# GmxMahdi/compute-raytracer

Measured on AMD Instinct MI355X. Metric: Mrays/s at 3840x2160, 1024 spheres, 8 bounces, higher is better.
Workload: dtype f32; 1 GPU; C3: 3840x2160, 1024 spheres (seed 358), 8 bounces, constant sky, reference default camera/light; mode=fast, variant=0, rays_per_frame=46143642, frames_in_flight=4, parallelism=row-tiles x1

## Files before the change

compute_raytracer_amd/abi.py:

```python
import ctypes
import os

_HERE = os.path.dirname(os.path.abspath(__file__))
LIB_PATH = os.environ.get("RT355_LIB") or os.path.join(_HERE, "librt355.so")

RT_OK = 0
RT_ERR_INVALID_ARG = -1
RT_ERR_NO_DEVICE = -2
RT_ERR_HIP = -3
RT_ERR_UNSUPPORTED = -4
RT_ERR_STATE = -5
RT_ERR_CAPACITY = -6
RT_ERR_COMM = -7
RT355_COMM_ID_BYTES = 128

RT_KERNEL_RAYTRACER = 0
RT_KERNEL_HEATMAP = 1
RT_MODE_FAST = 0
RT_MODE_STRICT = 1
RT_QUERY_LIMITS = 1

SYMBOLS = [
    "rt_create", "rt_destroy", "rt_last_error", "rt_abi_version", "rt_resize", "rt_write_params",
    "rt_write_spheres", "rt_write_cubemap_face", "rt_write_triangles", "rt_write_nodes", "rt_write_blas",
    "rt_write_tri_lookup", "rt_write_blas_lookup", "rt_write_mesh_texture", "rt_select_kernel", "rt_set_mode",
    "rt_set_variant", "rt_set_partition", "rt_tiles_of_rank", "rt_padded_tiles", "rt_render", "rt_wait",
    "rt_read_pixels", "rt_get_stats", "rt_render_to", "rt_assemble_frame", "rt_device_pixels",
    "rt_build_hierarchy", "rt_filter_plan", "rt_build_flow", "rt_order_tiles", "rt_read_hierarchy",
    "rt_comm_unique_id", "rt_comm_init", "rt_comm_destroy", "rt_render_gather", "rt_frame_pixels", "rt_read_frame",
    "rt_group_create", "rt_group_destroy", "rt_group_size", "rt_group_ctx", "rt_group_render", "rt_group_wait",
    "rt_build_id", "rt_kernel_name", "rt_set_comm_timeout",
    "rt_read_pixels_async", "rt_read_pixels_wait", "rt_host_alloc", "rt_host_free",
    "rt_trace_rays", "rt_trace_rays_host", "rt_pick",
    "rt_trace_rays_ex", "rt_trace_rays_host_ex", "rt_occluded", "rt_occluded_host",
]

KERNEL_IDS = {0: "none", 1: "literal", 2: "brute_single", 3: "brute_pipeline", 4: "hierarchy_8", 5: "hierarchy_12",
              6: "hierarchy_16", 7: "hierarchy_global", 8: "triangles", 9: "heatmap", 10: "triangles_roles"}


class RtStats(ctypes.Structure):
    _fields_ = [
        ("width", ctypes.c_uint32), ("height", ctypes.c_uint32), ("local_tiles", ctypes.c_uint32),
        ("spheres", ctypes.c_uint32), ("rays", ctypes.c_uint64), ("kernel_ms", ctypes.c_float),
        ("prep_ms", ctypes.c_float), ("frames", ctypes.c_uint32), ("mode", ctypes.c_int),
        ("batch_frames", ctypes.c_uint32), ("batch_kernel_ms", ctypes.c_float),
        ("gather_ms", ctypes.c_float), ("batch_gather_ms", ctypes.c_float),
        ("kernel_id", ctypes.c_uint32), ("grid_share", ctypes.c_uint32), ("instance_uploads", ctypes.c_uint32),
        ("tri_form", ctypes.c_uint32), ("pair_rebuilds", ctypes.c_uint32),
    ]


class RtHit(ctypes.Structure):
    _fields_ = [
        ("t", ctypes.c_float), ("u", ctypes.c_float), ("v", ctypes.c_float),
        ("prim", ctypes.c_int32), ("instance", ctypes.c_int32), ("normal", ctypes.c_float * 3),
    ]


HIT_DTYPE = [("t", "<f4"), ("u", "<f4"), ("v", "<f4"), ("prim", "<i4"), ("instance", "<i4"), ("normal", "<f4", (3,))]


class RtError(RuntimeError):
    def __init__(self, code, message):
        super().__init__("rt355 error %d: %s" % (code, message))
        self.code = code


_lib = None


def _one_hip_runtime():
    import sys
    if "torch" in sys.modules:
        return
    try:
        import importlib.util
        spec = importlib.util.find_spec("torch")
        if spec is None or not spec.submodule_search_locations:
            return
        cand = os.path.join(list(spec.submodule_search_locations)[0], "lib", "libamdhip64.so")
        if os.path.exists(cand):
            ctypes.CDLL(cand, mode=ctypes.RTLD_GLOBAL)
    except Exception:
        pass


def load():
    global _lib
    if _lib is not None:
        return _lib
    if not os.path.exists(LIB_PATH):
        raise RtError(RT_ERR_NO_DEVICE, "librt355.so is not built (%s); run `make lib`. There is no CPU path." % LIB_PATH)
    os.environ.setdefault("GPU_MAX_HW_QUEUES", "8")
    _one_hip_runtime()
    L = ctypes.CDLL(LIB_PATH)
    vp, u32, sz = ctypes.c_void_p, ctypes.c_uint32, ctypes.c_size_t
    fp = ctypes.POINTER(ctypes.c_float)
    sig = {
        "rt_create": (ctypes.c_int, [ctypes.c_int, ctypes.POINTER(vp)]),
        "rt_destroy": (ctypes.c_int, [vp]),
        "rt_last_error": (ctypes.c_char_p, [vp]),
        "rt_abi_version": (ctypes.c_int, []),
        "rt_resize": (ctypes.c_int, [vp, u32, u32]),
        "rt_write_params": (ctypes.c_int, [vp, fp]),
        "rt_write_spheres": (ctypes.c_int, [vp, fp, u32]),
        "rt_write_cubemap_face": (ctypes.c_int, [vp, ctypes.c_int, u32, u32, vp]),
        "rt_write_triangles": (ctypes.c_int, [vp, fp, u32]),
        "rt_write_nodes": (ctypes.c_int, [vp, sz, fp, u32]),
        "rt_write_blas": (ctypes.c_int, [vp, fp, u32]),
        "rt_write_tri_lookup": (ctypes.c_int, [vp, fp, u32]),
        "rt_write_blas_lookup": (ctypes.c_int, [vp, fp, u32]),
        "rt_write_mesh_texture": (ctypes.c_int, [vp, u32, u32, vp]),
        "rt_select_kernel": (ctypes.c_int, [vp, ctypes.c_int]),
        "rt_set_mode": (ctypes.c_int, [vp, ctypes.c_int]),
        "rt_set_variant": (ctypes.c_int, [vp, ctypes.c_int]),
        "rt_set_partition": (ctypes.c_int, [vp, u32, u32]),
        "rt_tiles_of_rank": (u32, [u32, u32, u32]),
        "rt_padded_tiles": (u32, [u32, u32]),
        "rt_render": (ctypes.c_int, [vp]),
        "rt_wait": (ctypes.c_int, [vp]),
        "rt_read_pixels": (ctypes.c_int, [vp, vp, sz]),
        "rt_get_stats": (ctypes.c_int, [vp, ctypes.POINTER(RtStats)]),
        "rt_render_to": (ctypes.c_int, [vp, vp, sz, vp]),
        "rt_assemble_frame": (ctypes.c_int, [vp, vp, vp, u32, vp]),
        "rt_device_pixels": (ctypes.c_int, [vp, ctypes.POINTER(vp), ctypes.POINTER(sz)]),
        "rt_build_hierarchy": (ctypes.c_int, [fp, u32, fp, ctypes.POINTER(u32), u32, ctypes.POINTER(u32)]),
        "rt_filter_plan": (ctypes.c_int, [fp, u32, fp, ctypes.POINTER(ctypes.c_int), ctypes.POINTER(ctypes.c_int)]),
        "rt_order_tiles": (ctypes.c_int, [vp, ctypes.POINTER(u32), u32, u32, ctypes.POINTER(u32), sz]),
        "rt_read_hierarchy": (ctypes.c_int, [vp, fp, ctypes.POINTER(u32), u32, ctypes.POINTER(u32)]),
        "rt_comm_unique_id": (ctypes.c_int, [vp]),
        "rt_comm_init": (ctypes.c_int, [vp, vp, u32, u32]),
        "rt_comm_destroy": (ctypes.c_int, [vp]),
        "rt_render_gather": (ctypes.c_int, [vp, ctypes.c_int]),
        "rt_frame_pixels": (ctypes.c_int, [vp, ctypes.POINTER(vp), ctypes.POINTER(sz)]),
        "rt_read_frame": (ctypes.c_int, [vp, vp, sz]),
        "rt_group_create": (ctypes.c_int, [ctypes.c_int, ctypes.POINTER(vp)]),
        "rt_group_destroy": (ctypes.c_int, [vp]),
        "rt_group_size": (ctypes.c_int, [vp]),
        "rt_group_ctx": (vp, [vp, ctypes.c_int]),
        "rt_group_render": (ctypes.c_int, [vp, ctypes.c_int]),
        "rt_group_wait": (ctypes.c_int, [vp]),
        "rt_build_id": (ctypes.c_char_p, []),
        "rt_kernel_name": (ctypes.c_char_p, [ctypes.c_int]),
        "rt_set_comm_timeout": (ctypes.c_int, [vp, u32]),
        "rt_read_pixels_async": (ctypes.c_int, [vp, u32, vp, sz]),
        "rt_read_pixels_wait": (ctypes.c_int, [vp]),
        "rt_host_alloc": (ctypes.c_int, [sz, ctypes.POINTER(vp)]),
        "rt_host_free": (ctypes.c_int, [vp]),
        "rt_trace_rays": (ctypes.c_int, [vp, vp, u32, vp, vp]),
        "rt_trace_rays_host": (ctypes.c_int, [vp, vp, u32, vp]),
        "rt_pick": (ctypes.c_int, [vp, vp, u32, vp]),
        "rt_trace_rays_ex": (ctypes.c_int, [vp, vp, u32, u32, vp, vp]),
        "rt_trace_rays_host_ex": (ctypes.c_int, [vp, vp, u32, u32, vp]),
        "rt_occluded": (ctypes.c_int, [vp, vp, u32, u32, vp, vp]),
        "rt_occluded_host": (ctypes.c_int, [vp, vp, u32, u32, vp]),
    }
    for name, (res, args) in sig.items():
        fn = getattr(L, name)
        fn.restype = res
        fn.argtypes = args
    _lib = L
    return L


def check(rc, ctx=None):
    if rc != RT_OK:
        msg = load().rt_last_error(ctx)
        raise RtError(rc, msg.decode("utf-8", "replace") if msg else "")
    return rc
```

compute_raytracer_amd/csrc/rt_api.hip:

```cpp
#include "rt_ctx.h"

#include <algorithm>
#include <cmath>
#include <condition_variable>
#include <mutex>
#include <thread>
#include <cstdio>
#include <cstdlib>
#include <cstring>
#include <new>
#include <string>
#include <vector>

#include "rt_bvh_build.h"
#include "rt_tlas_fit.h"

thread_local std::string g_rt_err;
thread_local int g_rt_kernel_id = 0;
thread_local int g_rt_tri_form = 0;

#ifndef RT355_BUILD_ID
#define RT355_BUILD_ID "unknown"
#endif

// ... 988 lines not shown
            RT_HIP(hipEventRecord(c->ev_k1[c->in_flight - 1u], st));
        }
#endif
    if (rc == RT_OK) { c->d_out = dst; c->buf_slot[k] = (int)c->in_flight - 1; ++c->frames_rendered; }
    return rc;
}

int rt_render_to(rt_ctx* c, void* device_dst, size_t cap, void* hip_stream) {
    if (!c || !device_dst) return fail(RT_ERR_INVALID_ARG, "rt_render_to: NULL argument");
    const size_t need = (size_t)local_tiles(c) * 8u * c->W * 4u;
    if (cap < need) return fail(RT_ERR_CAPACITY, "rt_render_to: destination smaller than local_tiles*8*W*4");
    hipStream_t s = hip_stream ? static_cast<hipStream_t>(hip_stream) : c->stream;
    return rt_enqueue(c, static_cast<uint8_t*>(device_dst), s);
}

void rt_abandon_in_flight(rt_ctx* c) {
    for (int k = 0; k < kStreams; ++k)
        if (c->streams[k]) (void)hipStreamSynchronize(c->streams[k]);
    if (c->in_flight) {
        (void)hipMemsetAsync(c->d_rays, 0, kCtrlBytes * c->in_flight, c->stream);
        (void)hipStreamSynchronize(c->stream);
    }
    (void)hipGetLastError();
    c->in_flight = 0;
    c->stats.batch_frames = 0;
    for (int v = 0; v < kVersions; ++v) c->ver_gen[v] = 0;
}

int rt_wait(rt_ctx* c) {
    if (!c) return fail(RT_ERR_INVALID_ARG, "rt_wait: ctx is NULL");
    RT_HIP(hipSetDevice(c->device));
    if (c->comm && c->in_flight) {
        int rc = rt_comm_wait_frames(c);
        if (rc != RT_OK) return rc;
    }
    for (uint32_t i = 0; i < c->in_flight; ++i) RT_HIP(hipEventSynchronize(c->ev_done[i]));
    if (c->in_flight) {
        c->stats.frames += c->in_flight;
        c->stats.rays = c->h_rays[2u * (c->in_flight - 1u)];
        c->stats.batch_frames = c->in_flight;
        {
            uint32_t distinct = 0;
            for (int k = 0; k < kStreams; ++k) {
                bool used = false;
                for (uint32_t i = 0; i < c->in_flight; ++i) used = used || c->slot_stream[i] == c->streams[k];
                distinct += used ? 1u : 0u;
            }
            c->pipelined_hint = distinct > 1u;
        }
        c->stats.batch_kernel_ms = 0.0f;
        for (uint32_t i = 0; i < c->in_flight; ++i) {
            float ms = 0.0f;
            if (hipEventElapsedTime(&ms, c->ev_k0[i], c->ev_k1[i]) == hipSuccess) {
                c->stats.kernel_ms = ms;
                c->stats.batch_kernel_ms += ms;
            }
            if (hipEventElapsedTime(&ms, c->ev_prep0[i], c->ev_k0[i]) == hipSuccess) c->stats.prep_ms = ms;
        }
        (void)hipGetLastError();
        c->in_flight = 0;
        for (int k = 0; k < kStreams; ++k) c->buf_slot[k] = -1;
        unsigned long long fault = 0ull;
        for (uint32_t i = 0; i < c->stats.batch_frames; ++i) fault = std::max(fault, c->h_rays[2u * i + 1u]);
        if (fault != 0ull) {
            char buf[160];
            std::snprintf(buf, sizeof buf, "rt_wait: the ray-trace kernel reported fault %llu (1: dynamic LDS not at address 0); the frame is incomplete", fault);
            g_rt_err = buf;
            return RT_ERR_HIP;
        }
        return rt_comm_after_wait(c);
    }
    return RT_OK;
}

int rt_read_pixels(rt_ctx* c, uint8_t* dst, size_t cap) {
    if (!c || !dst) return fail(RT_ERR_INVALID_ARG, "rt_read_pixels: NULL argument");
    if (!c->d_out) return fail(RT_ERR_STATE, "rt_read_pixels: no colour buffer (rt_resize first)");
    int rc = rt_wait(c);
    if (rc != RT_OK) return rc;
    const uint32_t lt = local_tiles(c);
    size_t rows = 0;
    for (uint32_t j = 0; j < lt; ++j) {
        const uint32_t y0 = (c->rank + j * c->world) * 8u;
        rows += (c->H - y0 >= 8u) ? 8u : (c->H - y0);
    }
    const size_t need = rows * c->W * 4u;
    if (cap < need) return fail(RT_ERR_CAPACITY, "rt_read_pixels: destination smaller than the local rows * W * 4");
    RT_HIP(hipMemcpyAsync(dst, c->d_out, need, hipMemcpyDeviceToHost, c->stream));
    RT_HIP(hipStreamSynchronize(c->stream));
    return RT_OK;
}

int rt_read_pixels_async(rt_ctx* c, uint32_t frames_back, uint8_t* dst, size_t cap) {
    if (!c || !dst) return fail(RT_ERR_INVALID_ARG, "rt_read_pixels_async: NULL argument");
    if (frames_back >= (uint32_t)kStreams || frames_back >= c->frames_rendered)
        return fail(RT_ERR_INVALID_ARG, "rt_read_pixels_async: frames_back must name one of the last four rt_render calls");
    if (c->world != 1u || c->comm) return fail(RT_ERR_STATE, "rt_read_pixels_async: whole-frame contexts only");
    if (!c->d_outs[0]) return fail(RT_ERR_STATE, "rt_read_pixels_async: no colour buffer (rt_resize first)");
    const size_t need = (size_t)c->H * c->W * 4u;
    if (cap < need) return fail(RT_ERR_CAPACITY, "rt_read_pixels_async: destination smaller than H * W * 4");
    RT_HIP(hipSetDevice(c->device));
    const uint32_t k = (c->frames_rendered - 1u - frames_back) % (uint32_t)kStreams;
    if (c->buf_slot[k] >= 0) RT_HIP(hipStreamWaitEvent(c->copy_stream, c->ev_k1[c->buf_slot[k]], 0));
    RT_HIP(hipMemcpyAsync(dst, c->d_outs[k], need, hipMemcpyDeviceToHost, c->copy_stream));
    RT_HIP(hipEventRecord(c->ev_copy[k], c->copy_stream));
    c->copy_pending[k] = true;
    return RT_OK;
}

int rt_read_pixels_wait(rt_ctx* c) {
    if (!c) return fail(RT_ERR_INVALID_ARG, "rt_read_pixels_wait: ctx is NULL");
    RT_HIP(hipSetDevice(c->device));
    RT_HIP(hipStreamSynchronize(c->copy_stream));
    for (int k = 0; k < kStreams; ++k) c->copy_pending[k] = false;
    return RT_OK;
}

int rt_host_alloc(size_t bytes, void** out) {
    if (!out || bytes == 0) return fail(RT_ERR_INVALID_ARG, "rt_host_alloc: NULL / zero size");
    *out = nullptr;
    RT_HIP(hipHostMalloc(out, bytes, hipHostMallocDefault));
    return RT_OK;
}

int rt_host_free(void* p) {
    if (p) RT_HIP(hipHostFree(p));
    return RT_OK;
}

int rt_get_stats(rt_ctx* c, rt_stats* out) {
    if (!c || !out) return fail(RT_ERR_INVALID_ARG, "rt_get_stats: NULL argument");
    c->stats.width = c->W;
    c->stats.height = c->H;
    c->stats.local_tiles = local_tiles(c);
    c->stats.spheres = c->n;
    c->stats.mode = c->mode;
    *out = c->stats;
    return RT_OK;
}

int rt_assemble_frame(rt_ctx* c, const void* gathered, void* frame, uint32_t world, void* hip_stream) {
    if (!c || !gathered || !frame) return fail(RT_ERR_INVALID_ARG, "rt_assemble_frame: NULL argument");
    if (world == 0) return fail(RT_ERR_INVALID_ARG, "rt_assemble_frame: world must be >= 1");
    if (!c->W || !c->H) return fail(RT_ERR_STATE, "rt_assemble_frame: rt_resize has not been called");
    RT_HIP(hipSetDevice(c->device));
    hipStream_t s = hip_stream ? static_cast<hipStream_t>(hip_stream) : c->stream;
    RT_HIP(rt_launch_assemble(static_cast<const uint8_t*>(gathered), static_cast<uint8_t*>(frame), c->W, c->H, world,
                              rt_padded_tiles(c->H, world), s));
    return RT_OK;
}

int rt_build_hierarchy(const float* records, uint32_t n, float* rec4, uint32_t* link, uint32_t cap_nodes,
                       uint32_t* n_nodes) {
    if ((n && !records) || !n_nodes) return fail(RT_ERR_INVALID_ARG, "rt_build_hierarchy: NULL argument");
    std::vector<float> r;
    std::vector<uint32_t> l;
    const uint32_t nodes = rt_bvh_build(records, n, r, l, rt_bvh_arity());
    *n_nodes = nodes;
    if (l.empty()) return RT_OK;
    if (cap_nodes < nodes + 1u || !rec4 || !link) return fail(RT_ERR_CAPACITY, "rt_build_hierarchy: need n_nodes + 1 entries");
    std::memcpy(rec4, r.data(), r.size() * sizeof(float));
    std::memcpy(link, l.data(), l.size() * sizeof(uint32_t));
    return RT_OK;
}

int rt_build_flow(const float* nodes, uint32_t n_nodes, const uint32_t* roots, uint32_t n_roots, float* pairs, uint32_t cap_pairs,
                  uint32_t* n_pairs, uint32_t* root_meta) {
    if (!nodes || (n_roots && !roots) || !n_pairs) return fail(RT_ERR_INVALID_ARG, "rt_build_flow: NULL argument");
    RtFlow f;
    rt_flow_build(nodes, n_nodes, roots, n_roots, f);
    *n_pairs = f.n_pairs;
    if (!f.ok) return fail(RT_ERR_UNSUPPORTED, "rt_build_flow: node buffer beyond 65,536 entries or a count beyond 16 bits");
    if (f.n_pairs && (cap_pairs < f.n_pairs || !pairs)) return fail(RT_ERR_CAPACITY, "rt_build_flow: need room for n_pairs records");
    if (f.n_pairs) std::memcpy(pairs, f.pairs.data(), (size_t)f.n_pairs * 64u);
    if (root_meta)
        for (uint32_t r = 0; r < n_roots; ++r)
            root_meta[r] = rt_flow_meta(nodes, n_nodes, roots[r] < n_nodes - 1u ? roots[r] : n_nodes - 1u, f.pair_of);
    return RT_OK;
}

int rt_order_tiles(rt_ctx* c, const uint32_t* cost, uint32_t n, uint32_t wave_slots, uint32_t* order, size_t cap) {
    if (!c || (n && !cost) || !order) return fail(RT_ERR_INVALID_ARG, "rt_order_tiles: NULL argument");
    if (cap < (size_t)n + 2u) return fail(RT_ERR_CAPACITY, "rt_order_tiles: order needs n + 2 entries");
    if (n > (1u << 26)) return fail(RT_ERR_INVALID_ARG, "rt_order_tiles: more than 2^26 tiles");
    order[0] = order[1] = 0u;
    if (n == 0u) return RT_OK;
    RT_HIP(hipSetDevice(c->device));
    const size_t cost_bytes = ((size_t)n * 4u + 7u) & ~(size_t)7u, scan_bytes = (size_t)rt_order_scan_words() * 4u;
    void *d_cost = nullptr, *d_order = nullptr;
    hipError_t e = hipMalloc(&d_cost, cost_bytes + scan_bytes);
    if (e == hipSuccess) e = hipMalloc(&d_order, ((size_t)n + 2u) * 4u);
    if (e == hipSuccess) e = hipMemsetAsync(d_cost, 0, cost_bytes + scan_bytes, c->stream);
    if (e == hipSuccess) e = hipMemcpyAsync(d_cost, cost, (size_t)n * 4u, hipMemcpyHostToDevice, c->stream);
    uint32_t* const scan = reinterpret_cast<uint32_t*>(static_cast<char*>(d_cost) + cost_bytes);
    for (int pass = 0; pass < 2 && e == hipSuccess; ++pass) {
        if (pass) e = hipMemcpyAsync(d_cost, cost, (size_t)n * 4u, hipMemcpyHostToDevice, c->stream);
        if (e == hipSuccess) e = rt_launch_order_hist(static_cast<uint32_t*>(d_cost), scan, static_cast<uint32_t*>(d_order), n, wave_slots, nullptr, nullptr, 0u, nullptr, c->stream);
        if (e == hipSuccess) e = rt_launch_order_scatter(static_cast<uint32_t*>(d_cost), scan, static_cast<uint32_t*>(d_order), n, c->stream);
    }
    if (e == hipSuccess) e = hipMemcpyAsync(order, d_order, ((size_t)n + 2u) * 4u, hipMemcpyDeviceToHost, c->stream);
    if (e == hipSuccess) e = hipStreamSynchronize(c->stream);
    (void)hipFree(d_cost);
    (void)hipFree(d_order);
    if (e != hipSuccess) return fail_hip(e, "rt_order_tiles");
    return RT_OK;
}

int rt_read_hierarchy(rt_ctx* c, float* rec4, uint32_t* link, uint32_t cap_nodes, uint32_t* n_nodes) {
    if (!c || !n_nodes) return fail(RT_ERR_INVALID_ARG, "rt_read_hierarchy: NULL argument");
    *n_nodes = 0;
    if (c->scene_kind != 0 || c->bvh_nodes == 0u || !c->d_bvh_rec || !c->d_bvh_link)
        return fail(RT_ERR_STATE, "rt_read_hierarchy: no frame of this sphere scene has walked a hierarchy");
    const uint32_t nodes = c->bvh_nodes;
    *n_nodes = nodes;
    if (cap_nodes < nodes + 1u || !rec4 || !link) return fail(RT_ERR_CAPACITY, "rt_read_hierarchy: need n_nodes + 1 entries");
    RT_HIP(hipSetDevice(c->device));
    { int rc = drain(c); if (rc != RT_OK) return rc; }
    const size_t nn = (size_t)nodes + 1u;
    RT_HIP(hipMemcpyAsync(rec4, c->d_bvh_rec, nn * sizeof(float4), hipMemcpyDeviceToHost, c->stream));
    RT_HIP(hipMemcpyAsync(link, c->d_bvh_link, nn * sizeof(uint32_t), hipMemcpyDeviceToHost, c->stream));
    RT_HIP(hipStreamSynchronize(c->stream));
    return RT_OK;
}

int rt_filter_plan(const float* records, uint32_t n, const float params[24], int* filter_ok, int* signed_filter) {
    if ((n && !records) || !params || !filter_ok || !signed_filter) return fail(RT_ERR_INVALID_ARG, "rt_filter_plan: NULL argument");
    bool ok = false;
    uint32_t sgn = 0;
    rt_plan((double)(float)rt_scene_bound(records, n), rt_scene_min_radius(records, n), params, ok, sgn);
    *filter_ok = ok ? 1 : 0;
    *signed_filter = (int)sgn;
    return RT_OK;
}


static int query_prepare(rt_ctx* c, const char* who, hipStream_t s, bool& tri, RtTriScene& ts, int& inst) {
    char msg[160];
    tri = c->scene_kind == 1;
    inst = 0;
    if (tri) {
        const bool have_blas = c->inst.blas_on ? !c->inst.blas.empty() : c->d_blas[0].used != 0;
        const bool have_lookup = c->inst.lookup_on ? !c->inst.lookup.empty() : c->d_blas_lookup[0].used != 0;
        if (!c->d_tri.used || !c->nodes_used || !have_blas || !c->d_tri_lookup.used || !have_lookup) {
            std::snprintf(msg, sizeof msg, "%s: a triangle scene needs rt_write_triangles, _nodes, _blas, _tri_lookup and _blas_lookup", who);
            return fail(RT_ERR_STATE, msg);
        }
    } else if (!c->have_spheres) {
        std::snprintf(msg, sizeof msg, "%s: no scene has been written", who);
        return fail(RT_ERR_STATE, msg);
    }
    RT_HIP(hipSetDevice(c->device));
    if (!c->ev_query) RT_HIP(hipEventCreateWithFlags(&c->ev_query, hipEventDisableTiming));
    if (tri) { int rc = ensure_corners(c, s); if (rc != RT_OK) return rc; }
    uint32_t v = 0;
    uint32_t root_meta[kInstMax] = {0};
    bool have_pairs = false;
    if (tri) {
        const uint32_t n_inst = (uint32_t)(c->inst.blas.size() / 20u);
        inst = (c->inst.blas_on && c->inst.lookup_on && n_inst >= 1u && c->inst.lookup.size() <= n_inst) ? 1 : 0;
        if (inst) {
            uint32_t roots[kInstMax], n_roots = 0;
            if (tri_pair_roots(c, roots, n_roots)) have_pairs = tri_pairs_current(c, roots, n_roots, root_meta);
        } else {
            int cur = -1;
            for (int k = 0; k < kVersions && cur < 0; ++k)
                if (c->ver_gen[k] == c->inst.gen) cur = k;
            if (cur < 0) {
                { int rc = drain(c); if (rc != RT_OK) return rc; }
                cur = 0;
                { int rc = apply_version(c, 0u, 0u, s); if (rc != RT_OK) return rc; }
            } else if (c->ev_ver[cur] && c->ver_stream[cur] != s) {
                RT_HIP(hipStreamWaitEvent(s, c->ev_ver[cur], 0));
            }
            v = (uint32_t)cur;
            c->query_versions = true;
        }
    }
    if (c->scene_stream && c->scene_stream != s) RT_HIP(hipStreamWaitEvent(s, c->ev_scene, 0));
    if (c->query_pending && c->query_last != s) RT_HIP(hipStreamWaitEvent(s, c->ev_query, 0));
    if (tri) {
        std::memset(&ts, 0, sizeof ts);
        tri_scene(c, v, have_pairs, root_meta, ts);
        if (inst) tri_fill_inst(c, ts);
    }
    return RT_OK;
}

static int query_launch(rt_ctx* c, const float4* rays, void* out, uint32_t n, hipStream_t s, bool tri, const RtTriScene& ts, int inst,
                        uint32_t flags = 0u, bool any = false) {
    if (!flags && !any) {
        float4* hits = static_cast<float4*>(out);
        if (tri) RT_HIP(rt_launch_query_triangles(ts, inst, rays, hits, n, s));
        else RT_HIP(rt_launch_query_spheres(c->d_records, c->n, rays, hits, n, s));
    } else {
        if (tri) RT_HIP(rt_launch_limited_triangles(ts, inst, rays, flags, any, out, n, s));
        else RT_HIP(rt_launch_limited_spheres(c->d_records, c->n, rays, flags, any, out, n, s));
    }
    RT_HIP(hipEventRecord(c->ev_query, s));
    c->query_pending = true;
    c->query_last = s;
    return RT_OK;
}

static int grow_staging(rt_ctx::DevBuf& b, size_t need) {
    if (need <= b.cap) return RT_OK;
    (void)hipFree(b.p);
    b.p = nullptr; b.cap = 0;
    const size_t cap = std::max(need, (size_t)65536u);
    RT_HIP(hipMalloc(&b.p, cap));
    b.cap = cap;
    return RT_OK;
// ... 112 lines not shown
```

compute_raytracer_amd/csrc/rt_bvh_build.h:

```cpp
#pragma once
#include <algorithm>
#include <cmath>
#include <cstdint>
#include <vector>

#ifndef RT_FILTER_KAPPA
#define RT_FILTER_KAPPA 1.52587890625e-05f
#define RT_FILTER_EPS 7.62939453125e-06f
#define RT_FILTER_SCALE 1099511627776.0f
#define RT_FILTER_SCALE2 1208925819614629174706176.0f
#endif
#ifndef RT_BVH_SIGMA
#define RT_BVH_SIGMA 1.04
#endif

namespace {

struct Builder {
    const float* rec;
    std::vector<float>& out_rec;
    std::vector<uint32_t>& out_link;
    std::vector<uint32_t> ids;
    uint32_t arity = 4;

    double cx(uint32_t i, int a) const {
        const double v = (double)rec[8u * (size_t)i + (size_t)a];
        return v == v ? v : 0.0;
    }
    double rad(uint32_t i) const {
        const double v = std::fabs((double)rec[8u * (size_t)i + 7u]);
        return v == v ? v : 0.0;
    }

    void leaf(uint32_t sphere) {
        out_rec.insert(out_rec.end(), {0.0f, 0.0f, 0.0f, 0.0f});
        out_link.push_back(0x80000000u | sphere);
    }

    uint32_t split2(uint32_t lo, uint32_t hi) {
        const uint32_t n = hi - lo;
        auto by_axis = [&](int ax) {
            return [this, ax](uint32_t a, uint32_t b) {
                const double va = cx(a, ax), vb = cx(b, ax);
                return va < vb || (va == vb && a < b);
            };
        };
        if (n > 32768u) {
            double mn[3] = {INFINITY, INFINITY, INFINITY}, mx[3] = {-INFINITY, -INFINITY, -INFINITY};
            for (uint32_t k = lo; k < hi; ++k)
                for (int a = 0; a < 3; ++a) {
                    const double v = cx(ids[k], a);
                    mn[a] = std::min(mn[a], v); mx[a] = std::max(mx[a], v);
                }
            int ax = 0;
            if (mx[1] - mn[1] > mx[ax] - mn[ax]) ax = 1;
            if (mx[2] - mn[2] > mx[ax] - mn[ax]) ax = 2;
            const uint32_t mid = lo + n / 2u;
            std::nth_element(ids.begin() + lo, ids.begin() + mid, ids.begin() + hi, by_axis(ax));
            return mid;
        }
        double best = INFINITY;
        int best_ax = 0;
        uint32_t best_k = n / 2u;
        std::vector<uint32_t> order(n);
        std::vector<double> suffix(n);
        for (int ax = 0; ax < 3; ++ax) {
            std::copy(ids.begin() + lo, ids.begin() + hi, order.begin());
            std::sort(order.begin(), order.end(), by_axis(ax));
            double mn[3] = {INFINITY, INFINITY, INFINITY}, mx[3] = {-INFINITY, -INFINITY, -INFINITY};
            auto grow = [&](uint32_t i) {
                double d2 = 0.0;
                for (int a = 0; a < 3; ++a) {
                    mn[a] = std::min(mn[a], cx(i, a) - rad(i));
                    mx[a] = std::max(mx[a], cx(i, a) + rad(i));
                    d2 += (mx[a] - mn[a]) * (mx[a] - mn[a]);
                }
                return d2;
            };
            for (uint32_t k = n; k-- > 1u;) suffix[k] = grow(order[k]) * (double)(n - k);
            for (int a = 0; a < 3; ++a) { mn[a] = INFINITY; mx[a] = -INFINITY; }
            for (uint32_t k = 1; k < n; ++k) {
                const double cost = grow(order[k - 1u]) * (double)k + suffix[k];
                if (cost < best) { best = cost; best_ax = ax; best_k = k; }
            }
        }
        std::sort(ids.begin() + lo, ids.begin() + hi, by_axis(best_ax));
        return lo + best_k;
    }

    void bound(uint32_t lo, uint32_t hi, float out[4]) {
        double mn[3] = {INFINITY, INFINITY, INFINITY}, mx[3] = {-INFINITY, -INFINITY, -INFINITY};
        for (uint32_t k = lo; k < hi; ++k)
            for (int a = 0; a < 3; ++a) {
                mn[a] = std::min(mn[a], cx(ids[k], a) - rad(ids[k]));
                mx[a] = std::max(mx[a], cx(ids[k], a) + rad(ids[k]));
            }
        auto radius_at = [&](const double P[3], uint32_t& far) {
            double R = -1.0;
            for (uint32_t k = lo; k < hi; ++k) {
                const uint32_t i = ids[k];
                const double dx = cx(i, 0) - P[0], dy = cx(i, 1) - P[1], dz = cx(i, 2) - P[2];
                const double d = std::sqrt(dx * dx + dy * dy + dz * dz) + rad(i);
                if (d > R) { R = d; far = i; }
            }
            return R;
        };
        double P[3] = {0.5 * (mn[0] + mx[0]), 0.5 * (mn[1] + mx[1]), 0.5 * (mn[2] + mx[2])};
        uint32_t far = ids[lo];
        double Rp = radius_at(P, far);
        for (int it = 0; it < 32; ++it) {
            const double s[3] = {cx(far, 0) - P[0], cx(far, 1) - P[1], cx(far, 2) - P[2]};
            const double len = std::sqrt(s[0] * s[0] + s[1] * s[1] + s[2] * s[2]);
            if (!(len > 1e-12)) break;
            const double Q[3] = {P[0] + s[0] / len * 0.05 * Rp, P[1] + s[1] / len * 0.05 * Rp, P[2] + s[2] / len * 0.05 * Rp};
            uint32_t far_q = far;
            const double Rq = radius_at(Q, far_q);
            if (!(Rq < Rp)) break;
            P[0] = Q[0]; P[1] = Q[1]; P[2] = Q[2]; Rp = Rq; far = far_q;
        }
        if (hi - lo > 2u) {
            double Q[3] = {P[0], P[1], P[2]};
            for (int it = 1; it <= 96; ++it) {
                uint32_t fq = far;
                const double Rq = radius_at(Q, fq);
                if (Rq < Rp) { Rp = Rq; P[0] = Q[0]; P[1] = Q[1]; P[2] = Q[2]; }
                const double s[3] = {cx(fq, 0) - Q[0], cx(fq, 1) - Q[1], cx(fq, 2) - Q[2]};
                const double len = std::sqrt(s[0] * s[0] + s[1] * s[1] + s[2] * s[2]);
                if (!(len > 1e-12)) break;
                const double k = (1.0 + rad(fq) / len) / (double)(it + 1);
                Q[0] += s[0] * k; Q[1] += s[1] * k; Q[2] += s[2] * k;
            }
        }
        const float C[3] = {(float)P[0], (float)P[1], (float)P[2]};
        const double Cd[3] = {C[0], C[1], C[2]};
        uint32_t unused = 0;
        double R = radius_at(Cd, unused);
        R *= RT_BVH_SIGMA;
        const double c2 = (double)C[0] * C[0] + (double)C[1] * C[1] + (double)C[2] * C[2];
        const double k = c2 * (1.0 - (double)RT_FILTER_EPS) - R * R * (1.0 + (double)RT_FILTER_KAPPA);
        out[0] = C[0] * RT_FILTER_SCALE; out[1] = C[1] * RT_FILTER_SCALE; out[2] = C[2] * RT_FILTER_SCALE;
        out[3] = (float)(k * (double)RT_FILTER_SCALE2);
    }

    void emit(uint32_t lo, uint32_t hi) {
        if (hi - lo == 1u) { leaf(ids[lo]); return; }
        const size_t me = out_link.size();
        out_rec.insert(out_rec.end(), {0.0f, 0.0f, 0.0f, 0.0f});
        out_link.push_back(0u);
        children(lo, hi);
        float b[4];
        bound(lo, hi, b);
        std::copy(b, b + 4, out_rec.begin() + 4 * me);
        out_link[me] = 4u * (uint32_t)out_link.size();
    }

    void children(uint32_t lo, uint32_t hi) {
        if (hi - lo <= arity) {
            for (uint32_t k = lo; k < hi; ++k) leaf(ids[k]);
            return;
        }
        uint32_t cut[9] = {lo, hi, 0, 0, 0, 0, 0, 0, 0};
        int parts = 1;
        while (parts < (int)arity) {
            int big = 0;
            for (int j = 1; j < parts; ++j)
                if (cut[j + 1] - cut[j] > cut[big + 1] - cut[big]) big = j;
            if (cut[big + 1] - cut[big] < 2u) break;
            const uint32_t mid = split2(cut[big], cut[big + 1]);
            for (int j = parts; j > big; --j) cut[j + 1] = cut[j];
            cut[big + 1] = mid;
            ++parts;
        }
        for (int j = 0; j < parts; ++j) emit(cut[j], cut[j + 1]);
    }
};

}

inline uint32_t rt_bvh_build(const float* records, uint32_t n, std::vector<float>& rec4, std::vector<uint32_t>& link, uint32_t arity = 4u) {
    rec4.clear(); link.clear();
    if (n == 0) return 0;
    rec4.reserve((size_t)n * 6u); link.reserve((size_t)n * 3u / 2u + 8u);
    Builder b{records, rec4, link, {}};
    b.arity = arity < 2u ? 2u : (arity > 8u ? 8u : arity);
    double mn[3] = {INFINITY, INFINITY, INFINITY}, mx[3] = {-INFINITY, -INFINITY, -INFINITY};
    for (uint32_t i = 0; i < n; ++i)
        for (int a = 0; a < 3; ++a) { mn[a] = std::min(mn[a], b.cx(i, a)); mx[a] = std::max(mx[a], b.cx(i, a)); }
    std::vector<double> radii(n);
    for (uint32_t i = 0; i < n; ++i) radii[i] = b.rad(i);
    std::nth_element(radii.begin(), radii.begin() + n / 2u, radii.end());
    const double med = radii[n / 2u];
    const double ext = std::sqrt((mx[0] - mn[0]) * (mx[0] - mn[0]) + (mx[1] - mn[1]) * (mx[1] - mn[1]) + (mx[2] - mn[2]) * (mx[2] - mn[2]));
    uint32_t big = 0;
    for (uint32_t i = 0; i < n; ++i) {
        const bool large = n > 8u && b.rad(i) > 8.0 * med && b.rad(i) > 0.125 * ext;
        if (large && big < 64u) { b.leaf(i); ++big; } else b.ids.push_back(i);
    }
    if (!b.ids.empty()) b.children(0u, (uint32_t)b.ids.size());
    const uint32_t nodes = (uint32_t)link.size();
    rec4.insert(rec4.end(), {0.0f, 0.0f, 0.0f, INFINITY});
    link.push_back(4u * nodes);
    return nodes;
}
```

include/rt355.h:

```cpp
#ifndef RT355_H
#define RT355_H

#include <stddef.h>
#include <stdint.h>

#ifdef __cplusplus
extern "C" {
#endif

#define RT355_ABI_VERSION 4

typedef enum rt_status {
    RT_OK = 0,
    RT_ERR_INVALID_ARG = -1,
    RT_ERR_NO_DEVICE = -2,
    RT_ERR_HIP = -3,
    RT_ERR_UNSUPPORTED = -4,
    RT_ERR_STATE = -5,
    RT_ERR_CAPACITY = -6,
    RT_ERR_COMM = -7
} rt_status;

typedef enum rt_kernel_id {
    RT_KID_NONE = 0,
    RT_KID_LITERAL = 1,
    RT_KID_BRUTE_SINGLE = 2,
    RT_KID_BRUTE_PIPELINE = 3,
    RT_KID_HIERARCHY_8 = 4,
    RT_KID_HIERARCHY_12 = 5,
    RT_KID_HIERARCHY_16 = 6,
    RT_KID_HIERARCHY_GLOBAL = 7,
    RT_KID_TRIANGLES = 8,
    RT_KID_HEATMAP = 9,
    RT_KID_TRIANGLES_ROLES = 10
} rt_kernel_id;

typedef enum rt_kernel {
    RT_KERNEL_RAYTRACER = 0,
    RT_KERNEL_HEATMAP = 1
} rt_kernel;

typedef enum rt_mode { RT_MODE_FAST = 0, RT_MODE_STRICT = 1 } rt_mode;

typedef struct rt_ctx rt_ctx;

typedef struct rt_stats {
    uint32_t width, height;
    uint32_t local_tiles;
    uint32_t spheres;
    uint64_t rays;
    float kernel_ms;
    float prep_ms;
    uint32_t frames;
    int mode;
    uint32_t batch_frames;
    float batch_kernel_ms;
    float gather_ms;
    float batch_gather_ms;
    uint32_t kernel_id;
    uint32_t grid_share;
    uint32_t instance_uploads;
    uint32_t tri_form;
    uint32_t pair_rebuilds;
} rt_stats;


int rt_create(int device, rt_ctx** out);
int rt_destroy(rt_ctx* ctx);

const char* rt_last_error(rt_ctx* ctx);

int rt_abi_version(void);

const char* rt_build_id(void);
const char* rt_kernel_name(int kernel_id);


int rt_resize(rt_ctx* ctx, uint32_t width, uint32_t height);

int rt_write_params(rt_ctx* ctx, const float params[24]);

int rt_write_spheres(rt_ctx* ctx, const float* records, uint32_t n);

int rt_write_cubemap_face(rt_ctx* ctx, int face, uint32_t w, uint32_t h, const uint8_t* rgba);

int rt_write_triangles(rt_ctx* ctx, const float* data, uint32_t n_triangles);
int rt_write_nodes(rt_ctx* ctx, size_t byte_offset, const float* data, uint32_t n);
int rt_write_blas(rt_ctx* ctx, const float* data, uint32_t n_blas);
int rt_write_tri_lookup(rt_ctx* ctx, const float* data, uint32_t n);
int rt_write_blas_lookup(rt_ctx* ctx, const float* data, uint32_t n);
int rt_write_mesh_texture(rt_ctx* ctx, uint32_t w, uint32_t h, const uint8_t* rgba);

int rt_select_kernel(rt_ctx* ctx, int kernel);

int rt_set_mode(rt_ctx* ctx, int mode);

int rt_set_variant(rt_ctx* ctx, int variant);


int rt_set_partition(rt_ctx* ctx, uint32_t rank, uint32_t world);

uint32_t rt_tiles_of_rank(uint32_t height, uint32_t rank, uint32_t world);
uint32_t rt_padded_tiles(uint32_t height, uint32_t world);


#define RT355_MAX_IN_FLIGHT 64
int rt_render(rt_ctx* ctx);

int rt_wait(rt_ctx* ctx);

int rt_read_pixels(rt_ctx* ctx, uint8_t* dst, size_t cap);

int rt_read_pixels_async(rt_ctx* ctx, uint32_t frames_back, uint8_t* dst, size_t cap);
int rt_read_pixels_wait(rt_ctx* ctx);
int rt_host_alloc(size_t bytes, void** out);
int rt_host_free(void* p);

int rt_get_stats(rt_ctx* ctx, rt_stats* out);


int rt_render_to(rt_ctx* ctx, void* device_dst, size_t cap, void* hip_stream);

int rt_assemble_frame(rt_ctx* ctx, const void* gathered, void* frame, uint32_t world,
                      void* hip_stream);

int rt_device_pixels(rt_ctx* ctx, void** out_ptr, size_t* out_bytes);


typedef struct rt_hit {
    float t;
    float u, v;
    int32_t prim;
    int32_t instance;
    float normal[3];
} rt_hit;

int rt_trace_rays(rt_ctx* ctx, const float* rays, uint32_t n, rt_hit* hits, void* hip_stream);
int rt_trace_rays_host(rt_ctx* ctx, const float* rays, uint32_t n, rt_hit* hits);
int rt_pick(rt_ctx* ctx, const uint32_t* xy, uint32_t n, rt_hit* hits);


#define RT_QUERY_LIMITS 1u

int rt_trace_rays_ex(rt_ctx* ctx, const float* rays, uint32_t n, uint32_t flags, rt_hit* hits, void* hip_stream);
int rt_trace_rays_host_ex(rt_ctx* ctx, const float* rays, uint32_t n, uint32_t flags, rt_hit* hits);
int rt_occluded(rt_ctx* ctx, const float* rays, uint32_t n, uint32_t flags, uint8_t* occluded, void* hip_stream);
int rt_occluded_host(rt_ctx* ctx, const float* rays, uint32_t n, uint32_t flags, uint8_t* occluded);


#define RT355_COMM_ID_BYTES 128
int rt_comm_unique_id(uint8_t id[RT355_COMM_ID_BYTES]);
int rt_comm_init(rt_ctx* ctx, const uint8_t id[RT355_COMM_ID_BYTES], uint32_t rank, uint32_t world);
int rt_comm_destroy(rt_ctx* ctx);

int rt_set_comm_timeout(rt_ctx* ctx, uint32_t ms);

int rt_render_gather(rt_ctx* ctx, int root);

int rt_frame_pixels(rt_ctx* ctx, void** out_ptr, size_t* out_bytes);
int rt_read_frame(rt_ctx* ctx, uint8_t* dst, size_t cap);

typedef struct rt_group rt_group;
int rt_group_create(int n_devices, rt_group** out);
int rt_group_destroy(rt_group* g);
int rt_group_size(const rt_group* g);
rt_ctx* rt_group_ctx(rt_group* g, int i);
int rt_group_render(rt_group* g, int root);
int rt_group_wait(rt_group* g);


int rt_build_hierarchy(const float* records, uint32_t n, float* rec4, uint32_t* link, uint32_t cap_nodes,
                       uint32_t* n_nodes);

int rt_build_flow(const float* nodes, uint32_t n_nodes, const uint32_t* roots, uint32_t n_roots, float* pairs, uint32_t cap_pairs,
                  uint32_t* n_pairs, uint32_t* root_meta);

int rt_order_tiles(rt_ctx* ctx, const uint32_t* cost, uint32_t n, uint32_t wave_slots, uint32_t* order, size_t cap);

int rt_read_hierarchy(rt_ctx* ctx, float* rec4, uint32_t* link, uint32_t cap_nodes, uint32_t* n_nodes);

int rt_filter_plan(const float* records, uint32_t n, const float params[24], int* filter_ok, int* signed_filter);

#ifdef __cplusplus
}
#endif
#endif
```

Before: 31140 Mrays/s.

## Add reinsertion optimisation pass to sphere BVH builder

After the top-down build, the BVH builder now keeps an explicit node tree and runs a reinsertion optimiser. It detaches subtrees under the largest parents, searches for cheaper placements using a bounding-ball cost, and keeps moves that lower the cost, with journaled rollback. Emitted bounds are recomputed for dirty nodes, and the result is discarded if the final cost rises. The aim is a tighter hierarchy so traversal visits fewer nodes per ray, at the price of extra host build time and more complex builder code.

```diff
diff --git a/compute_raytracer_amd/abi.py b/compute_raytracer_amd/abi.py
--- a/compute_raytracer_amd/abi.py
+++ b/compute_raytracer_amd/abi.py
@@ -33,6 +33,7 @@
     "rt_read_pixels_async", "rt_read_pixels_wait", "rt_host_alloc", "rt_host_free",
     "rt_trace_rays", "rt_trace_rays_host", "rt_pick",
     "rt_trace_rays_ex", "rt_trace_rays_host_ex", "rt_occluded", "rt_occluded_host",
+    "rt_build_hierarchy_ex",
 ]
 
 KERNEL_IDS = {0: "none", 1: "literal", 2: "brute_single", 3: "brute_pipeline", 4: "hierarchy_8", 5: "hierarchy_12",
@@ -126,6 +127,8 @@
         "rt_assemble_frame": (ctypes.c_int, [vp, vp, vp, u32, vp]),
         "rt_device_pixels": (ctypes.c_int, [vp, ctypes.POINTER(vp), ctypes.POINTER(sz)]),
         "rt_build_hierarchy": (ctypes.c_int, [fp, u32, fp, ctypes.POINTER(u32), u32, ctypes.POINTER(u32)]),
+        "rt_build_hierarchy_ex": (ctypes.c_int, [fp, u32, fp, ctypes.POINTER(u32), u32, ctypes.POINTER(u32), u32,
+                                                 ctypes.POINTER(ctypes.c_double)]),
         "rt_filter_plan": (ctypes.c_int, [fp, u32, fp, ctypes.POINTER(ctypes.c_int), ctypes.POINTER(ctypes.c_int)]),
         "rt_order_tiles": (ctypes.c_int, [vp, ctypes.POINTER(u32), u32, u32, ctypes.POINTER(u32), sz]),
         "rt_read_hierarchy": (ctypes.c_int, [vp, fp, ctypes.POINTER(u32), u32, ctypes.POINTER(u32)]),
diff --git a/compute_raytracer_amd/csrc/rt_api.hip b/compute_raytracer_amd/csrc/rt_api.hip
--- a/compute_raytracer_amd/csrc/rt_api.hip
+++ b/compute_raytracer_amd/csrc/rt_api.hip
@@ -1164,11 +1164,18 @@
 
 int rt_build_hierarchy(const float* records, uint32_t n, float* rec4, uint32_t* link, uint32_t cap_nodes,
                        uint32_t* n_nodes) {
+    return rt_build_hierarchy_ex(records, n, rec4, link, cap_nodes, n_nodes, RT355_HIERARCHY_PASSES, nullptr);
+}
+
+int rt_build_hierarchy_ex(const float* records, uint32_t n, float* rec4, uint32_t* link, uint32_t cap_nodes,
+                          uint32_t* n_nodes, uint32_t passes, double* info) {
     if ((n && !records) || !n_nodes) return fail(RT_ERR_INVALID_ARG, "rt_build_hierarchy: NULL argument");
     std::vector<float> r;
     std::vector<uint32_t> l;
-    const uint32_t nodes = rt_bvh_build(records, n, r, l, rt_bvh_arity());
+    rt_bvh_build_info bi;
+    const uint32_t nodes = rt_bvh_build(records, n, r, l, rt_bvh_arity(), passes > 16u ? 16u : passes, &bi);
     *n_nodes = nodes;
+    if (info) { info[0] = (double)bi.nodes_topdown; info[1] = (double)bi.moves; info[2] = bi.cost_topdown; info[3] = bi.cost; }
     if (l.empty()) return RT_OK;
     if (cap_nodes < nodes + 1u || !rec4 || !link) return fail(RT_ERR_CAPACITY, "rt_build_hierarchy: need n_nodes + 1 entries");
     std::memcpy(rec4, r.data(), r.size() * sizeof(float));
diff --git a/compute_raytracer_amd/csrc/rt_bvh_build.h b/compute_raytracer_amd/csrc/rt_bvh_build.h
--- a/compute_raytracer_amd/csrc/rt_bvh_build.h
+++ b/compute_raytracer_amd/csrc/rt_bvh_build.h
@@ -2,6 +2,7 @@
 #include <algorithm>
 #include <cmath>
 #include <cstdint>
+#include <utility>
 #include <vector>
 
 #ifndef RT_FILTER_KAPPA
@@ -88,7 +89,7 @@
         return lo + best_k;
     }
 
-    void bound(uint32_t lo, uint32_t hi, float out[4]) {
+    void bound(uint32_t lo, uint32_t hi, float out[4], double* sphere = nullptr) {
         double mn[3] = {INFINITY, INFINITY, INFINITY}, mx[3] = {-INFINITY, -INFINITY, -INFINITY};
         for (uint32_t k = lo; k < hi; ++k)
             for (int a = 0; a < 3; ++a) {
@@ -135,6 +136,7 @@
         const double Cd[3] = {C[0], C[1], C[2]};
         uint32_t unused = 0;
         double R = radius_at(Cd, unused);
+        if (sphere) { sphere[0] = Cd[0]; sphere[1] = Cd[1]; sphere[2] = Cd[2]; sphere[3] = R; }
         R *= RT_BVH_SIGMA;
         const double c2 = (double)C[0] * C[0] + (double)C[1] * C[1] + (double)C[2] * C[2];
         const double k = c2 * (1.0 - (double)RT_FILTER_EPS) - R * R * (1.0 + (double)RT_FILTER_KAPPA);
@@ -142,21 +144,49 @@
         out[3] = (float)(k * (double)RT_FILTER_SCALE2);
     }
 
-    void emit(uint32_t lo, uint32_t hi) {
-        if (hi - lo == 1u) { leaf(ids[lo]); return; }
-        const size_t me = out_link.size();
-        out_rec.insert(out_rec.end(), {0.0f, 0.0f, 0.0f, 0.0f});
-        out_link.push_back(0u);
-        children(lo, hi);
+    static constexpr uint32_t ROOT = 0xFFFFFFFFu;
+    struct Node {
+        uint32_t parent = ROOT, nk = 0, sphere = 0;
+        uint32_t kid[8] = {0, 0, 0, 0, 0, 0, 0, 0};
+        double s[4] = {0.0, 0.0, 0.0, 0.0};
+        float rec[4] = {0.0f, 0.0f, 0.0f, 0.0f};
+        double r_rec = 0.0;
+        bool dirty = false;
+        bool fixed = false;
+        bool dead = false;
+    };
+    std::vector<Node> nodes;
+    std::vector<uint32_t> top;
+
+    uint32_t new_leaf(uint32_t sphere, uint32_t parent) {
+        Node l;
+        l.parent = parent; l.sphere = sphere;
+        l.s[0] = cx(sphere, 0); l.s[1] = cx(sphere, 1); l.s[2] = cx(sphere, 2); l.s[3] = rad(sphere);
+        nodes.push_back(l);
+        return (uint32_t)nodes.size() - 1u;
+    }
+    void add_kid(uint32_t parent, uint32_t k) {
+        if (parent == ROOT) top.push_back(k); else nodes[parent].kid[nodes[parent].nk++] = k;
+    }
+
+    uint32_t make(uint32_t lo, uint32_t hi, uint32_t parent) {
+        if (hi - lo == 1u) return new_leaf(ids[lo], parent);
+        const uint32_t me = (uint32_t)nodes.size();
+        nodes.emplace_back();
+        nodes[me].parent = parent;
+        children(lo, hi, me);
         float b[4];
-        bound(lo, hi, b);
-        std::copy(b, b + 4, out_rec.begin() + 4 * me);
-        out_link[me] = 4u * (uint32_t)out_link.size();
-    }
-
-    void children(uint32_t lo, uint32_t hi) {
+        double s[4];
+        bound(lo, hi, b, s);
+        std::copy(b, b + 4, nodes[me].rec);
+        std::copy(s, s + 4, nodes[me].s);
+        nodes[me].r_rec = s[3];
+        return me;
+    }
+
+    void children(uint32_t lo, uint32_t hi, uint32_t parent) {
         if (hi - lo <= arity) {
-            for (uint32_t k = lo; k < hi; ++k) leaf(ids[k]);
+            for (uint32_t k = lo; k < hi; ++k) add_kid(parent, new_leaf(ids[k], parent));
             return;
         }
         uint32_t cut[9] = {lo, hi, 0, 0, 0, 0, 0, 0, 0};
@@ -171,14 +201,266 @@
             cut[big + 1] = mid;
             ++parts;
         }
-        for (int j = 0; j < parts; ++j) emit(cut[j], cut[j + 1]);
+        for (int j = 0; j < parts; ++j) {
+            const uint32_t k = make(cut[j], cut[j + 1], parent);
+            add_kid(parent, k);
+        }
+    }
+
+    static double ball_cost(const Node& x) { return x.nk ? x.s[3] * x.s[3] * (double)x.nk : 0.0; }
+    static double rec_cost(const Node& x) { return x.nk ? x.r_rec * x.r_rec * (double)x.nk : 0.0; }
+    void emit(uint32_t node, double& cost) {
+        if (nodes[node].nk == 0u) { ids.push_back(nodes[node].sphere); leaf(nodes[node].sphere); return; }
+        const size_t me = out_link.size();
+        const uint32_t first = (uint32_t)ids.size();
+        out_rec.insert(out_rec.end(), {0.0f, 0.0f, 0.0f, 0.0f});
+        out_link.push_back(0u);
+        for (uint32_t k = 0; k < nodes[node].nk; ++k) emit(nodes[node].kid[k], cost);
+        if (nodes[node].dirty) {
+            bound(first, (uint32_t)ids.size(), nodes[node].rec, nodes[node].s);
+            nodes[node].r_rec = nodes[node].s[3];
+            nodes[node].dirty = false;
+        }
+        cost += rec_cost(nodes[node]);
+        std::copy(nodes[node].rec, nodes[node].rec + 4, out_rec.begin() + 4 * me);
+        out_link[me] = 4u * (uint32_t)out_link.size();
+    }
+    double emit_all() {
+        out_rec.clear(); out_link.clear(); ids.clear();
+        double cost = 0.0;
+        for (uint32_t t : top) emit(t, cost);
+        return cost;
+    }
+
+    std::vector<std::pair<uint32_t, Node>> journal;
+    std::vector<std::pair<uint32_t, uint32_t>> top_journal;
+    std::vector<uint32_t> stamp;
+    std::vector<std::pair<double, uint32_t>> search_heap;
+    uint32_t txn = 0, inner_live = 0;
+
+    void touch(uint32_t i) {
+        if (stamp.size() < nodes.size()) stamp.resize(nodes.size(), 0u);
+        if (stamp[i] == txn) return;
+        stamp[i] = txn;
+        journal.emplace_back(i, nodes[i]);
+    }
+    static void merge2(const double a[4], const double b[4], double o[4]) {
+        const double d[3] = {b[0] - a[0], b[1] - a[1], b[2] - a[2]};
+        const double len = std::sqrt(d[0] * d[0] + d[1] * d[1] + d[2] * d[2]);
+        if (len + b[3] <= a[3]) { const double t[4] = {a[0], a[1], a[2], a[3]}; std::copy(t, t + 4, o); return; }
+        if (len + a[3] <= b[3]) { const double t[4] = {b[0], b[1], b[2], b[3]}; std::copy(t, t + 4, o); return; }
+        const double R = 0.5 * (len + a[3] + b[3]);
+        const double f = len > 0.0 ? (R - a[3]) / len : 0.0;
+        const double t[4] = {a[0] + d[0] * f, a[1] + d[1] * f, a[2] + d[2] * f, R};
+        std::copy(t, t + 4, o);
+    }
+    void kids_ball(const Node& x, double o[4]) const {
+        std::copy(nodes[x.kid[0]].s, nodes[x.kid[0]].s + 4, o);
+        for (uint32_t k = 1; k < x.nk; ++k) merge2(o, nodes[x.kid[k]].s, o);
+        if (x.nk < 3u) return;
+        double q[3] = {o[0], o[1], o[2]};
+        for (int it = 1; it <= 8; ++it) {
+            double R = -1.0, len_f = 0.0;
+            uint32_t far = 0;
+            for (uint32_t k = 0; k < x.nk; ++k) {
+                const double* c = nodes[x.kid[k]].s;
+                const double len = std::sqrt((c[0] - q[0]) * (c[0] - q[0]) + (c[1] - q[1]) * (c[1] - q[1]) + (c[2] - q[2]) * (c[2] - q[2]));
+                if (len + c[3] > R) { R = len + c[3]; far = k; len_f = len; }
+            }
+            if (R < o[3]) { o[0] = q[0]; o[1] = q[1]; o[2] = q[2]; o[3] = R; }
+            if (!(len_f > 1e-300)) break;
+            const double* c = nodes[x.kid[far]].s;
+            const double f = (1.0 + c[3] / len_f) / (double)(it + 1);
+            q[0] += (c[0] - q[0]) * f; q[1] += (c[1] - q[1]) * f; q[2] += (c[2] - q[2]) * f;
+        }
+    }
+    void refit_up(uint32_t x, const double* added) {
+        for (; x != ROOT; x = nodes[x].parent) {
+            double alt[4], nb[4];
+            if (added) merge2(nodes[x].s, added, alt); else std::copy(nodes[x].s, nodes[x].s + 4, alt);
+            kids_ball(nodes[x], nb);
+            const double* pick = nb[3] < alt[3] ? nb : alt;
+            if (pick[0] == nodes[x].s[0] && pick[1] == nodes[x].s[1] && pick[2] == nodes[x].s[2] && pick[3] == nodes[x].s[3]) {
+                if (!added) break;
+                continue;
+            }
+            touch(x);
+            std::copy(pick, pick + 4, nodes[x].s);
+        }
+    }
+    void replace_kid(uint32_t parent, uint32_t was, uint32_t now) {
+        if (parent == ROOT) {
+            for (uint32_t k = 0; k < (uint32_t)top.size(); ++k)
+                if (top[k] == was) { top_journal.emplace_back(k, was); top[k] = now; return; }
+            return;
+        }
+        touch(parent);
+        for (uint32_t k = 0; k < nodes[parent].nk; ++k)
+            if (nodes[parent].kid[k] == was) { nodes[parent].kid[k] = now; return; }
+    }
+    void detach(uint32_t s) {
+        const uint32_t p = nodes[s].parent;
+        touch(p); touch(s);
+        Node& P = nodes[p];
+        uint32_t w = 0;
+        for (uint32_t k = 0; k < P.nk; ++k) if (P.kid[k] != s) P.kid[w++] = P.kid[k];
+        P.nk = w;
+        nodes[s].parent = ROOT;
+        uint32_t from = p;
+        if (P.nk == 1u) {
+            const uint32_t q = P.kid[0], g = P.parent;
+            touch(q);
+            nodes[q].parent = g;
+            replace_kid(g, p, q);
+            nodes[p].nk = 0; nodes[p].dead = true;
+            --inner_live;
+            from = g;
+        }
+        refit_up(from, nullptr);
+    }
+    bool find_place(uint32_t s, bool allow_pair, bool allow_child, uint32_t& where, bool& pair) {
+        typedef std::pair<double, uint32_t> Item;
+        auto later = [](const Item& a, const Item& b) { return a.first > b.first || (a.first == b.first && a.second > b.second); };
+        std::vector<Item>& heap = search_heap;
+        heap.clear();
+        for (uint32_t t : top)
+            if (!nodes[t].fixed) { heap.emplace_back(0.0, t); std::push_heap(heap.begin(), heap.end(), later); }
+        double best = INFINITY;
+        bool found = false;
+        const double* S = nodes[s].s;
+        int budget = 256;
+        while (!heap.empty() && budget-- > 0) {
+            std::pop_heap(heap.begin(), heap.end(), later);
+            const Item it = heap.back();
+            heap.pop_back();
+            if (!(it.first < best)) break;
+            const Node& X = nodes[it.second];
+            double m[4];
+            merge2(X.s, S, m);
+            const double m2 = m[3] * m[3];
+            if (allow_pair) {
+                const double c = it.first + 2.0 * m2;
+                if (c < best) { best = c; where = it.second; pair = true; found = true; }
+            }
+            if (X.nk) {
+                const double down = it.first + (m2 - X.s[3] * X.s[3]) * (double)X.nk;
+                if (allow_child && X.nk < arity && down + m2 < best) { best = down + m2; where = it.second; pair = false; found = true; }
+                if (down < best)
+                    for (uint32_t k = 0; k < X.nk; ++k) { heap.emplace_back(down, X.kid[k]); std::push_heap(heap.begin(), heap.end(), later); }
+            }
+        }
+        return found;
+    }
+    void attach(uint32_t s, uint32_t where, bool pair) {
+        double S[4];
+        std::copy(nodes[s].s, nodes[s].s + 4, S);
+        touch(s);
+        if (!pair) {
+            touch(where);
+            nodes[where].kid[nodes[where].nk++] = s;
+            nodes[s].parent = where;
+            refit_up(where, S);
+            return;
+        }
+        const uint32_t g = nodes[where].parent;
+        const uint32_t nn = (uint32_t)nodes.size();
+        nodes.emplace_back();
+        Node& N = nodes[nn];
+        N.parent = g; N.nk = 2; N.kid[0] = where; N.kid[1] = s; N.dirty = true;
+        merge2(nodes[where].s, S, N.s);
+        replace_kid(g, where, nn);
+        touch(where);
+        nodes[where].parent = nn;
+        nodes[s].parent = nn;
+        ++inner_live;
+        refit_up(g, S);
+    }
+    void mark_dirty(uint32_t from, uint32_t to) {
+        ++txn;
+        if (stamp.size() < nodes.size()) stamp.resize(nodes.size(), 0u);
+        for (uint32_t x = to; x != ROOT; x = nodes[x].parent) stamp[x] = txn;
+        uint32_t lca = from;
+        while (lca != ROOT && stamp[lca] != txn) { nodes[lca].dirty = true; lca = nodes[lca].parent; }
+        for (uint32_t x = to; x != lca; x = nodes[x].parent) nodes[x].dirty = true;
+    }
+    uint32_t optimise(uint32_t passes) {
+        uint32_t inner_topdown = 0;
+        for (const Node& x : nodes) inner_topdown += x.nk ? 1u : 0u;
+        inner_live = inner_topdown;
+        uint32_t moves = 0;
+        std::vector<std::pair<double, uint32_t>> cand;
+        for (uint32_t pass = 0; pass < passes; ++pass) {
+            cand.clear();
+            for (uint32_t i = 0; i < (uint32_t)nodes.size(); ++i) {
+                const Node& x = nodes[i];
+                if (x.dead || x.parent == ROOT) continue;
+                const double r = nodes[x.parent].s[3];
+                cand.emplace_back(r == r ? r : 0.0, i);
+            }
+            std::sort(cand.begin(), cand.end(), [](const std::pair<double, uint32_t>& a, const std::pair<double, uint32_t>& b) {
+                return a.first > b.first || (a.first == b.first && a.second < b.second);
+            });
+            const size_t tries = (cand.size() + 1u) / 2u;
+            uint32_t kept = 0;
+            for (size_t ci = 0; ci < tries; ++ci) {
+                const auto& cd = cand[ci];
+                const uint32_t s = cd.second;
+                if (nodes[s].dead || nodes[s].parent == ROOT) continue;
+                uint32_t depth = 0;
+                for (uint32_t a = nodes[s].parent; a != ROOT && depth <= 64u; a = nodes[a].parent) ++depth;
+                if (depth > 64u) continue;
+                ++txn;
+                journal.clear(); top_journal.clear();
+                const size_t size0 = nodes.size();
+                const uint32_t live0 = inner_live, old_parent = nodes[s].parent;
+                detach(s);
+                uint32_t where = 0;
+                bool pair = false;
+                const bool dissolved = inner_live < live0;
+                bool ok = find_place(s, dissolved, !dissolved, where, pair);
+                if (ok && !pair && where == old_parent && !nodes[old_parent].dead) ok = false;
+                double delta = 0.0;
+                if (ok) {
+                    attach(s, where, pair);
+                    for (const auto& j : journal) delta += ball_cost(nodes[j.first]) - ball_cost(j.second);
+                    for (size_t i = size0; i < nodes.size(); ++i) delta += ball_cost(nodes[i]);
+                }
+                if (ok && delta < 0.0) {
+                    mark_dirty(old_parent, nodes[s].parent);
+                    ++moves; ++kept;
+                } else {
+                    nodes.resize(size0);
+                    for (size_t i = journal.size(); i-- > 0;) nodes[journal[i].first] = journal[i].second;
+                    for (size_t i = top_journal.size(); i-- > 0;) top[top_journal[i].first] = top_journal[i].second;
+                    inner_live = live0;
+                }
+            }
+            if (!kept) break;
+        }
+        return moves;
     }
 };
 
 }
 
-inline uint32_t rt_bvh_build(const float* records, uint32_t n, std::vector<float>& rec4, std::vector<uint32_t>& link, uint32_t arity = 4u) {
+#ifndef RT_BVH_OPT_PASSES
+#ifdef RT355_HIERARCHY_PASSES
+#define RT_BVH_OPT_PASSES RT355_HIERARCHY_PASSES
+#else
+#define RT_BVH_OPT_PASSES 1u
+#endif
+#endif
+
+struct rt_bvh_build_info {
+    uint32_t nodes_topdown = 0;
+    uint32_t moves = 0;
+    double cost_topdown = 0.0, cost = 0.0;
+};
+
+inline uint32_t rt_bvh_build(const float* records, uint32_t n, std::vector<float>& rec4, std::vector<uint32_t>& link, uint32_t arity = 4u,
+                             uint32_t passes = RT_BVH_OPT_PASSES, rt_bvh_build_info* info = nullptr) {
     rec4.clear(); link.clear();
+    if (info) *info = rt_bvh_build_info();
     if (n == 0) return 0;
     rec4.reserve((size_t)n * 6u); link.reserve((size_t)n * 3u / 2u + 8u);
     Builder b{records, rec4, link, {}};
@@ -191,13 +473,46 @@
     std::nth_element(radii.begin(), radii.begin() + n / 2u, radii.end());
     const double med = radii[n / 2u];
     const double ext = std::sqrt((mx[0] - mn[0]) * (mx[0] - mn[0]) + (mx[1] - mn[1]) * (mx[1] - mn[1]) + (mx[2] - mn[2]) * (mx[2] - mn[2]));
+    b.nodes.reserve((size_t)n * 2u + 8u);
     uint32_t big = 0;
     for (uint32_t i = 0; i < n; ++i) {
         const bool large = n > 8u && b.rad(i) > 8.0 * med && b.rad(i) > 0.125 * ext;
-        if (large && big < 64u) { b.leaf(i); ++big; } else b.ids.push_back(i);
-    }
-    if (!b.ids.empty()) b.children(0u, (uint32_t)b.ids.size());
+        if (large && big < 64u) {
+            const uint32_t l = b.new_leaf(i, Builder::ROOT);
+            b.nodes[l].fixed = true;
+            b.top.push_back(l);
+            ++big;
+        } else b.ids.push_back(i);
+    }
+    const uint32_t rest = (uint32_t)b.ids.size();
+    if (rest) b.children(0u, rest, Builder::ROOT);
+    double cost0 = 0.0;
+    bool finite = true;
+    for (const Builder::Node& x : b.nodes) {
+        cost0 += Builder::rec_cost(x);
+        finite = finite && std::isfinite(x.s[0]) && std::isfinite(x.s[1]) && std::isfinite(x.s[2]) && std::isfinite(x.s[3]);
+    }
+    const uint32_t nodes_topdown = (uint32_t)b.nodes.size();
+    uint32_t moves = 0;
+    double cost = cost0;
+    if (passes && rest <= 32768u && finite && std::isfinite(cost0)) {
+        const std::vector<Builder::Node> nodes0 = b.nodes;
+        const std::vector<uint32_t> top0 = b.top;
+        moves = b.optimise(passes);
+        if (moves) {
+            cost = b.emit_all();
+            if (!(cost <= cost0) || link.size() > nodes0.size()) {
+                b.nodes = nodes0; b.top = top0;
+                moves = 0;
+                cost = b.emit_all();
+            }
+        } else cost = b.emit_all();
+    } else cost = b.emit_all();
     const uint32_t nodes = (uint32_t)link.size();
+    if (info) {
+        info->nodes_topdown = nodes_topdown;
+        info->moves = moves; info->cost_topdown = cost0; info->cost = cost;
+    }
     rec4.insert(rec4.end(), {0.0f, 0.0f, 0.0f, INFINITY});
     link.push_back(4u * nodes);
     return nodes;
diff --git a/include/rt355.h b/include/rt355.h
--- a/include/rt355.h
+++ b/include/rt355.h
@@ -172,6 +172,10 @@
 int rt_build_hierarchy(const float* records, uint32_t n, float* rec4, uint32_t* link, uint32_t cap_nodes,
                        uint32_t* n_nodes);
 
+#define RT355_HIERARCHY_PASSES 1u
+int rt_build_hierarchy_ex(const float* records, uint32_t n, float* rec4, uint32_t* link, uint32_t cap_nodes,
+                          uint32_t* n_nodes, uint32_t passes, double* info);
+
 int rt_build_flow(const float* nodes, uint32_t n_nodes, const uint32_t* roots, uint32_t n_roots, float* pairs, uint32_t cap_pairs,
                   uint32_t* n_pairs, uint32_t* root_meta);
 
```

Measured after the change: 31480 Mrays/s, median of 6. 1.01x the previous value.
